# uricchio/2DSFS-scan

Measured on AMD Instinct MI355X. Metric: genomic windows/s (T2D+T1D+Fst) at 20 kb, n1=n2=50; HBM GB/s fraction, higher is better.
Workload: dtype f64

## Files before the change

### 2dsfs-scan_amd/csrc/sfs2d.hip

```cpp
#include <hip/hip_runtime.h>
#include <hip/hip_ext.h>

#include <algorithm>
#include <cmath>
#include <cstdint>
#include <cstdio>
#include <cstdlib>
#include <cstring>
#include <string>
#include <mutex>
#include <vector>

#include "sfs2d.h"
#include "sfs2d_kernels.hpp"

using namespace sfs2dk;

namespace {

struct PwTree {
  std::vector<int2> leaves;
  std::vector<int4> nodes;
  int nlevels = 0;
};
// ... 45 lines not shown

#define CTX_STREAM(c) ((c)->stream)

struct sfs2d_ctx {
  int device = 0;
  int ncu = 256;
  hipStream_t own = nullptr;
  hipStream_t stream = nullptr;
  double* d_lnx = nullptr;
  double* d_df = nullptr;
  hipEvent_t stagger = nullptr;
  std::string err;
  std::mutex err_mu;
};

struct sfs2d_data {
  sfs2d_ctx* ctx = nullptr;
  bool owned = false;
  uint32_t* counts = nullptr;
  uint32_t* pos = nullptr;
  uint16_t* ann = nullptr;
  long long* d_chrom_off = nullptr;
  int64_t n = 0;
  int32_t nchrom = 0;
  std::vector<int64_t> chrom_off;
  std::vector<uint32_t> last_pos;
  std::vector<uint32_t> host_pos;
  bool ann_owned = false;
  bool strict = true;
  uint32_t max_nc1 = 0xffffffffu, max_nc2 = 0xffffffffu;
  bool low_nc = true;
  unsigned long long* d_win_off = nullptr;
  uint32_t win_bp = 0, win_per_chrom = 0;
};

struct sfs2d_plan {
  sfs2d_ctx* ctx = nullptr;
  const sfs2d_data* data = nullptr;
  sfs2d_params prm{};
  KParams K{};
  int nbg = 0;
  bool do_bg = false, do_seg = false, lds_hist = true, bg_ready = false;
  bool seg_synth = false;
  bool seg_search = false;
  int64_t step = 0;
  bool fused = false;
  bool sliced = false;
  bool cnt = false;
  bool fst = false;
  double* d_fst = nullptr;
  double* d_fst_own = nullptr;
  unsigned long long* d_fsum = nullptr;
  int hr = 1;
  uint64_t runs = 0;
  int G = 64;
  bool gw = false;
  uint32_t* d_gscr = nullptr;
  int nscr = 0;
  bool p16 = true;
  size_t scan_lds = 0, bg_lds = 0, extra_lds = 0;
  int64_t nslots = 0, nrec = 0, extra_rec = -1;
  uint32_t last_chrom = 0;
  std::vector<Tile> tiles;
  std::vector<Chunk> chunks;
  std::vector<int4> slices;
  Tile* d_tiles = nullptr;
  Chunk* d_chunks = nullptr;
  uint2* d_slots = nullptr;
  uint32_t* d_repl = nullptr;
  uint32_t* d_bcount = nullptr;
  uint32_t* d_done = nullptr;
  uint32_t* d_ctr = nullptr;
  double* d_bgval = nullptr;
  PL* d_tab = nullptr;
  double* d_lp = nullptr;
  BgHead* d_head = nullptr;
  Bg1D* d_bg1d = nullptr;
// ... 217 lines not shown
template <bool B, bool S, bool L, bool N>
hipError_t launch_prep1(sfs2d_plan* pl) {
  const bool f = pl->K.ann_want >= 0 || pl->K.has_start || pl->K.has_end;
  return f ? launch_prep2<B, S, L, N, true>(pl) : launch_prep2<B, S, L, N, false>(pl);
}

hipError_t launch_prep_cnt(sfs2d_plan* pl) {
  const bool L = pl->lds_hist;
  const bool fs = pl->fst && !pl->fst_win && !pl->fst_scan;
  if (pl->do_bg && pl->do_seg)
    return L ? launch_prep1<true, true, true, false>(pl) : launch_prep1<true, true, false, false>(pl);
  if (pl->do_bg) return L ? launch_prep1<true, false, true, false>(pl) : launch_prep1<true, false, false, false>(pl);
  if (pl->do_seg) return launch_prep1<false, true, false, false>(pl);
  if (fs) return launch_prep1<false, false, false, false>(pl);
  return hipSuccess;
}

bool slots_only(const sfs2d_plan* pl) {
  return (pl->seg_synth || pl->seg_search) && pl->attached.empty() && !(pl->fst && !pl->fst_win && !pl->fst_scan);
}

hipError_t launch_slots_only(sfs2d_plan* pl) {
  const unsigned long long nw = (unsigned long long)pl->nslots;
  if (nw && pl->seg_synth)
    hipExtLaunchKernelGGL(k_slots_synth, dim3((unsigned)std::min<unsigned long long>(8192, (nw + 255) / 256)), dim3(256),
                          0, CTX_STREAM(pl->ctx), pl->kev[0], pl->kev[1], 0, pl->data->d_win_off, nw, pl->d_slots);
  else if (nw)
    hipExtLaunchKernelGGL(k_slots_search, dim3((unsigned)((nw + 255) / 256)), dim3(256), 0, CTX_STREAM(pl->ctx),
                          pl->kev[0], pl->kev[1], 0, pl->data->pos, pl->data->d_chrom_off, pl->d_slot_base,
                          pl->data->nchrom, (uint32_t)pl->prm.window, (uint32_t)nw, pl->d_slots);
  return hipGetLastError();
}

bool prep_runs(const sfs2d_plan* pl) {
  return !pl->tiles.empty() && (!pl->cnt || pl->do_bg || pl->do_seg || (pl->fst && !pl->fst_win && !pl->fst_scan));
}

hipError_t launch_slots_slide(sfs2d_plan* pl, bool ev) {
  const uint32_t ns = (uint32_t)pl->nslots;
  if (!ns) return hipSuccess;
  hipExtLaunchKernelGGL(k_slots_slide, dim3((ns + 255u) / 256u), dim3(256), 0, CTX_STREAM(pl->ctx), ev ? pl->kev[0] : nullptr,
                        ev ? pl->kev[1] : nullptr, 0, pl->data->pos, pl->data->d_chrom_off, pl->d_slot_base, pl->data->nchrom,
                        (uint32_t)pl->prm.window, (uint32_t)pl->step, ns, pl->d_slots);
  return hipGetLastError();
}

hipError_t launch_fst_win(sfs2d_plan* a) {
  const uint32_t ns = (uint32_t)a->nslots;
  if (!ns) return hipSuccess;
  const dim3 gf((unsigned)std::min<uint32_t>(2048u, (ns + 3u) / 4u));
  if (a->cnt)
    hipLaunchKernelGGL(k_fst_win<true>, gf, dim3(256), 0, CTX_STREAM(a->ctx), a->K, a->data->counts, scan_src(a), a->d_slots,
                       reinterpret_cast<const double2*>(a->ctx->d_df + 2 * LNT), a->d_fst, ns);
  else
    hipLaunchKernelGGL(k_fst_win<false>, gf, dim3(256), 0, CTX_STREAM(a->ctx), a->K, a->data->counts, scan_src(a), a->d_slots,
                       reinterpret_cast<const double2*>(a->ctx->d_df + 2 * LNT), a->d_fst, ns);
  return hipGetLastError();
}

hipError_t launch_prep(sfs2d_plan* pl, bool bins) {
  if (pl->tiles.empty()) return hipSuccess;
  const bool L = pl->lds_hist;
  if (!bins) return L ? launch_prep1<true, false, true, false>(pl) : launch_prep1<true, false, false, false>(pl);
  if (pl->cnt) return launch_prep_cnt(pl);
  if (pl->do_bg && pl->do_seg)
    return L ? launch_prep1<true, true, true, true>(pl) : launch_prep1<true, true, false, true>(pl);
// ... 307 lines not shown
  if (e != hipSuccess) {
    hipFree(d_woff);
    hipFree(d->counts); hipFree(d->pos); hipFree(d->ann); hipFree(d->d_chrom_off); delete d;
    return set_err(ctx, SFS2D_E_HIP, std::string("synthetic data: ") + hipGetErrorString(e));
  }
  d->d_win_off = d_woff;
  d->win_bp = sp->window_bp;
  d->win_per_chrom = sp->n_windows;
  d->last_pos.assign(sp->n_replicates, sp->n_windows * sp->window_bp);
  d->strict = true;
  d->max_nc1 = 2u * (uint32_t)sp->n1p;
  d->max_nc2 = 2u * (uint32_t)sp->n2p;
  *out = d;
  return 0;
}

int sfs2d_data_read(const sfs2d_data* d, uint32_t* counts, uint32_t* pos, int64_t n) {
  if (!d || n != d->n) return SFS2D_E_ARG;
  sfs2d_ctx* ctx = d->ctx;
  HIPCHK(ctx, hipSetDevice(ctx->device));
  HIPCHK(ctx, hipStreamSynchronize(CTX_STREAM(ctx)));
  if (counts && n) HIPCHK(ctx, hipMemcpy(counts, d->counts, sizeof(uint32_t) * (size_t)n, hipMemcpyDeviceToHost));
  if (pos && n) HIPCHK(ctx, hipMemcpy(pos, d->pos, sizeof(uint32_t) * (size_t)n, hipMemcpyDeviceToHost));
  return 0;
}

int sfs2d_data_free(sfs2d_data* d) {
  if (!d) return SFS2D_E_ARG;
  hipSetDevice(d->ctx->device);
  if (d->owned) { hipFree(d->counts); hipFree(d->pos); }
  if (d->owned || d->ann_owned) hipFree(d->ann);
  hipFree(d->d_chrom_off);
  hipFree(d->d_win_off);
  delete d;
  return 0;
}

static int make_kparams(sfs2d_ctx* ctx, const sfs2d_params* prm, int nchrom, KParams* K) {
  *K = KParams{};
  if (!prm) return set_err(ctx, SFS2D_E_ARG, "params is NULL");
  if (prm->n1p < 1 || prm->n2p < 1 || 2 * prm->n1p > 255 || 2 * prm->n2p > 255)
    return set_err(ctx, SFS2D_E_ARG, "pop sizes must satisfy 1 <= pop_size and 2*pop_size <= 255 (u8 counts)");
  if (prm->window_mode != SFS2D_WINDOW_BP && prm->window_mode != SFS2D_WINDOW_SNPS)
    return set_err(ctx, SFS2D_E_ARG, "bad window_mode");
  if (prm->window < 1 || prm->window > 0xffffffffll) return set_err(ctx, SFS2D_E_ARG, "window must be in [1, 2^32)");
  if (prm->bg_mode != SFS2D_BG_PER_CHROM && prm->bg_mode != SFS2D_BG_SUPPLIED) return set_err(ctx, SFS2D_E_ARG, "bad bg_mode");
  K->n1p = prm->n1p; K->n2p = prm->n2p; K->n1 = 2 * prm->n1p; K->n2 = 2 * prm->n2p;
  K->nb2 = (K->n1 + 1) * (K->n2 + 1);
  K->h1a = K->nb2; K->h1b = K->nb2 + K->n1 + 1; K->nh = (K->h1b + K->n2 + 1 + 3) & ~3;
  K->t1a = K->nb2; K->t1b = K->nb2 + K->n1p + 1; K->nt = K->t1b + K->n2p + 1;
  K->rtn = wl_rtn(K->n1p, K->n2p);
  K->fold = prm->fold ? 1 : 0;
  K->fold_thr = prm->fold ? K->n1p + K->n2p : 0x7fffffff;
  K->ann_want = prm->ann_want;
  K->has_start = prm->has_start ? 1 : 0; K->has_end = prm->has_end ? 1 : 0;
  K->start_pos = prm->start_pos; K->end_pos = prm->end_pos;
  K->ws = (unsigned)prm->window;
  div_magic(K->ws, &K->wmag, &K->wsh1, &K->wsh2);
  K->nchrom = nchrom;
  K->fst_e = 40;
  K->fst_scale = std::ldexp(1.0, K->fst_e);
  return 0;
}

static int plan_create(sfs2d_ctx* ctx, const sfs2d_data* data, const sfs2d_params* prm, int force_sliced, int64_t step,
                       sfs2d_plan** out);

// ... 193 lines not shown
        if (const char* ev = std::getenv("SFS2D_GW")) pl->gw = occ >= 1 && ev[0] == '1';
      }
      if (pl->gw) pl->scan_lds = gw_lds;
    }
  }
  if (pl->scan_lds > 160 * 1024) {
    delete pl;
    return set_err(ctx, SFS2D_E_ARG, "2D grid too large for LDS with 32-bit bins (windows of >= 65536 SNPs)");
  }
  const bool small = pl->do_bg && pl->G == WAVE;
  const double wpw = (double)pl->nslots / (2.0 * ctx->ncu * (SBLOCK / WAVE));
  pl->sliced = small && wpw < 4.0;
  if (const char* ev = std::getenv("SFS2D_FUSED")) pl->sliced = small && ev[0] == '0';
  if (force_sliced >= 0) pl->sliced = small && force_sliced == 1;
  pl->fused = small && !pl->sliced;
  pl->fst = (prm->flags & SFS2D_F_FST) != 0;
  pl->fst_scan = false;
  if (pl->fst && pl->cnt && pl->G == WAVE && !pl->gw) {
    const char* ev = std::getenv("SFS2D_FST_SCAN");
    pl->fst_scan = !(ev && ev[0] == '0');
    if (pl->fst_scan) {
      hipFuncAttributes fa{};
      const void* f = pl->p16 ? (const void*)k_scan_w<true, true, 2, true> : (const void*)k_scan_w<false, true, 2, true>;
      if (hipFuncGetAttributes(&fa, f) != hipSuccess || pl->scan_lds + fa.sharedSizeBytes > 160 * 1024) pl->fst_scan = false;
    }
  }
  pl->gate = pl->fst_scan && prm->fold && nc_ok;
  pl->lean = pl->gate && bp && K.n1p <= 31 && K.n2p <= 31;
  if (const char* ev = std::getenv("SFS2D_LEAN")) pl->lean = pl->lean && ev[0] != '0';
  const PwTree pw = pw_plan(K.nb2 - 3);
  pl->fst_mask = data->low_nc;
  pl->fst_win = pl->sliced && bp && pl->fst && !pl->fst_scan;
  if (slide) pl->fst_win = pl->fst && !pl->fst_scan;
  pl->nfst = pl->fst_win && !slide ? (int)std::min<int64_t>(1024, std::max<int64_t>(1, (pl->nslots + 7) / 8)) : 0;
  if (pl->scan_lds > 64 * 1024) {
    const int lds = (int)pl->scan_lds;
    const hipFuncAttribute A = hipFuncAttributeMaxDynamicSharedMemorySize;
    for (const void* f : {(const void*)k_scan_w<true, true, false, false>, (const void*)k_scan_w<false, true, false, false>,
                          (const void*)k_scan_w<true, false, false, false>, (const void*)k_scan_w<false, false, false, false>,
                          (const void*)k_scan_w<true, true, true, false>, (const void*)k_scan_w<false, true, true, false>,
                          (const void*)k_scan_w<true, false, true, false>, (const void*)k_scan_w<false, false, true, false>,
                          (const void*)k_scan_w<true, true, false, true>, (const void*)k_scan_w<false, true, false, true>,
                          (const void*)k_scan_w<true, false, false, true>, (const void*)k_scan_w<false, false, false, true>,
                          (const void*)k_scan_w<true, true, true, true>, (const void*)k_scan_w<false, true, true, true>,
                          (const void*)k_scan_w<true, false, true, true>, (const void*)k_scan_w<false, false, true, true>,
                          (const void*)k_scan_w<true, true, 2, true>, (const void*)k_scan_w<false, true, 2, true>,
                          (const void*)k_scan_w<true, false, 2, true>, (const void*)k_scan_w<false, false, 2, true>,
                          (const void*)k_scan_w<true, true, 3, true>, (const void*)k_scan_w<false, true, 3, true>,
                          (const void*)k_scan_w<true, false, 3, true>, (const void*)k_scan_w<false, false, 3, true>,
                          (const void*)k_scan_w<true, true, 2, true, true>, (const void*)k_scan_w<false, true, 2, true, true>,
                          (const void*)k_scan_w<true, false, 2, true, true>, (const void*)k_scan_w<false, false, 2, true, true>,
                          (const void*)k_scan_w<true, true, 3, true, true>, (const void*)k_scan_w<false, true, 3, true, true>,
                          (const void*)k_scan_w<true, false, 3, true, true>, (const void*)k_scan_w<false, false, 3, true, true>,
                          (const void*)k_scan_w<true, true, 2, true, true, true>, (const void*)k_scan_w<false, true, 2, true, true, true>,
                          (const void*)k_scan_w<true, false, 2, true, true, true>, (const void*)k_scan_w<false, false, 2, true, true, true>,
                          (const void*)k_scan_w<true, true, 3, true, true, true>, (const void*)k_scan_w<false, true, 3, true, true, true>,
                          (const void*)k_scan_w<true, false, 3, true, true, true>, (const void*)k_scan_w<false, false, 3, true, true, true>,
                          (const void*)k_scan_g<true, false, false>, (const void*)k_scan_g<false, false, false>,
                          (const void*)k_scan_g<true, true, false>, (const void*)k_scan_g<false, true, false>,
                          (const void*)k_scan_g<true, false, true>, (const void*)k_scan_g<false, false, true>,
                          (const void*)k_scan_g<true, true, true>, (const void*)k_scan_g<false, true, true>})
      hipFuncSetAttribute(f, A, lds);
  }
  if (pl->extra_lds > 64 * 1024) {
    for (const void* f : {(const void*)k_scan_extra<true, false>, (const void*)k_scan_extra<false, false>,
                          (const void*)k_scan_extra<true, true>, (const void*)k_scan_extra<false, true>})
// ... 157 lines not shown
    const int ke = jl == pl->nleaves ? K.nb2 : 1 + pw.leaves[jl].x;
    pl->slices.push_back(make_int4(kb, ke, j, jl));
  }
  if (pl->slices.empty()) pl->slices.push_back(make_int4(0, K.nb2, 0, 0));

  hipStream_t st = CTX_STREAM(ctx);
  rc = 0;
  rc = rc ? rc : dalloc(ctx, &pl->d_tiles, pl->tiles.size());
  rc = rc ? rc : dalloc(ctx, &pl->d_chunks, pl->chunks.size());
  rc = rc ? rc : dalloc(ctx, &pl->d_slots, (size_t)pl->nslots + 1);
  const size_t nrepl = pl->do_bg ? (size_t)(pl->fused ? 2 : 1) * REPL * nc * K.nh : 1;
  rc = rc ? rc : dalloc(ctx, &pl->d_repl, nrepl);
  rc = rc ? rc : dalloc(ctx, &pl->d_bcount, (size_t)2 * std::max(1, nc));
  rc = rc ? rc : dalloc(ctx, &pl->d_done, (size_t)pl->nbg);
  const size_t nctr = (size_t)2 * std::max(1, nc) * CTR_POOLS * CTR_STRIDE;
  rc = rc ? rc : dalloc(ctx, &pl->d_ctr, nctr);
  const size_t ngscr = pl->gw ? (size_t)pl->nscr * (K.nb2 + 1) : 0;
  if (pl->gw) rc = rc ? rc : dalloc(ctx, &pl->d_gscr, ngscr);
  rc = rc ? rc : dalloc(ctx, &pl->d_bgval, (size_t)pl->nbg * K.nt);
  rc = rc ? rc : dalloc(ctx, &pl->d_tab, (size_t)pl->nbg * K.nt);
  rc = rc ? rc : dalloc(ctx, &pl->d_lp, (size_t)pl->nbg * K.nt);
  rc = rc ? rc : dalloc(ctx, &pl->d_head, (size_t)pl->nbg);
  rc = rc ? rc : dalloc(ctx, &pl->d_bg1d, (size_t)pl->nbg);
  rc = rc ? rc : dalloc(ctx, &pl->d_leafsum, (size_t)pl->nbg * std::max(1, pl->nleaves));
  rc = rc ? rc : dalloc(ctx, &pl->d_leaves, pw.leaves.size());
  rc = rc ? rc : dalloc(ctx, &pl->d_nodes, pw.nodes.size());
  rc = rc ? rc : dalloc(ctx, &pl->d_slices, pl->slices.size());
  const size_t nbins = pl->cnt ? 4 : ((size_t)data->n + 3) / 4 * 4 + SCAN_PAD;
  rc = rc ? rc : dalloc(ctx, &pl->d_bins, nbins);
  rc = rc ? rc : dalloc(ctx, &pl->d_out, (size_t)pl->nrec);
  rc = rc ? rc : dalloc(ctx, &pl->d_err, 4);
  if (pl->fst) rc = rc ? rc : dalloc(ctx, &pl->d_fst, (size_t)pl->nslots + 1);
  pl->d_fst_own = pl->d_fst;
  if ((pl->seg_search || slide) && !rc) {
    std::vector<uint32_t> sb(pl->slot_base_h.begin(), pl->slot_base_h.end());
    rc = dalloc(ctx, &pl->d_slot_base, sb.size());
    if (!rc && hipMemcpy(pl->d_slot_base, sb.data(), sizeof(uint32_t) * sb.size(), hipMemcpyHostToDevice) != hipSuccess)
      rc = set_err(ctx, SFS2D_E_HIP, "slot bases upload");
  }
  if (pl->fst) rc = rc ? rc : dalloc(ctx, &pl->d_fsum, 2 * ((size_t)pl->nslots + 1));
  if (rc) { plan_free(pl); delete pl; return rc; }
  hipError_t e = hipSuccess;
#define PCPY(dst, v) if (e == hipSuccess && !(v).empty()) e = hipMemcpyAsync(dst, (v).data(), sizeof((v)[0]) * (v).size(), hipMemcpyHostToDevice, st)
  PCPY(pl->d_tiles, pl->tiles);
  PCPY(pl->d_chunks, pl->chunks);
  PCPY(pl->d_leaves, pw.leaves);
  PCPY(pl->d_nodes, pw.nodes);
  PCPY(pl->d_slices, pl->slices);
#undef PCPY
  if (e == hipSuccess) e = hipMemsetAsync(pl->d_slots, 0, sizeof(uint2) * ((size_t)pl->nslots + 1), st);
  if (e == hipSuccess && pl->do_bg) e = hipMemsetAsync(pl->d_repl, 0, sizeof(uint32_t) * nrepl, st);
  if (e == hipSuccess) e = hipMemsetAsync(pl->d_bcount, 0, sizeof(uint32_t) * 2 * std::max(1, nc), st);
  if (e == hipSuccess) e = hipMemsetAsync(pl->d_done, 0, sizeof(uint32_t) * pl->nbg, st);
  if (e == hipSuccess) e = hipMemsetAsync(pl->d_ctr, 0, sizeof(uint32_t) * nctr, st);
  if (e == hipSuccess && pl->gw) e = hipMemsetAsync(pl->d_gscr, 0, sizeof(uint32_t) * ngscr, st);
  if (e == hipSuccess) e = hipMemsetAsync(pl->d_err, 0, 4 * sizeof(uint32_t), st);
  if (e == hipSuccess) e = hipMemsetAsync(pl->d_bins, 0, sizeof(uint32_t) * nbins, st);
  if (e == hipSuccess && pl->fst) e = hipMemsetAsync(pl->d_fsum, 0, sizeof(unsigned long long) * 2 * ((size_t)pl->nslots + 1), st);
  if (e == hipSuccess) e = hipMemsetAsync(pl->d_out, 0, sizeof(sfs2d_window) * (size_t)pl->nrec, st);
  for (auto& ev : pl->ev) if (e == hipSuccess) e = hipEventCreate(&ev);
  if (e == hipSuccess) e = hipStreamSynchronize(st);
  if (e != hipSuccess) {
    plan_free(pl); delete pl;
    return set_err(ctx, SFS2D_E_HIP, std::string("plan setup: ") + hipGetErrorString(e));
  }
  pl->bg_ready = false;
  *out = pl;
// ... 20 lines not shown
  HIPCHK(ctx, hipStreamSynchronize(CTX_STREAM(ctx)));
  pl->bg_ready = true;
  return 0;
}

int sfs2d_plan_run_phase(sfs2d_plan* pl, int phase, sfs2d_window* out_dev) {
  if (!pl) return SFS2D_E_ARG;
  sfs2d_ctx* ctx = pl->ctx;
  if (pl->base) return set_err(ctx, SFS2D_E_ARG, "an attached plan runs with its base plan (sfs2d_plan_attach)");
  HIPCHK(ctx, hipSetDevice(ctx->device));
  hipEvent_t* te = nullptr;
  if (phase == 2) {
    te = pl->tpend;
    pl->tpend = nullptr;
  } else if (pl->timing && (pl->tseen++ % pl->tevery) == 0 && pl->tcount < pl->tmax) {
    te = &pl->tev[(size_t)pl->tcount * 6];
  }
  if (!pl->do_bg && !pl->bg_ready && phase != 1)
    return set_err(ctx, SFS2D_E_ARG, "supplied-background plan run before sfs2d_plan_set_background");
  for (int k = 0; k < 6; ++k) pl->kev[k] = (te && ((pl->tmask >> (k / 2)) & 1)) ? te[k] : nullptr;
  auto mark = [&](int k) -> int {
    if (te && ((pl->tmask >> (k / 2)) & 1)) {
      HIPCHK(ctx, hipEventRecord(te[k], CTX_STREAM(ctx)));
      HIPCHK(ctx, hipEventRecord(te[k + 1], CTX_STREAM(ctx)));
    }
    return 0;
  };
  int rc = 0;
  if (phase == 0 || phase == 1) {
    if (slots_only(pl)) {
      HIPCHK(ctx, launch_slots_only(pl));
      if (pl->nslots == 0 && (rc = mark(0))) return rc;
    } else {
      HIPCHK(ctx, launch_prep(pl, true));
      const bool slots = pl->step && pl->nslots;
      if (slots) HIPCHK(ctx, launch_slots_slide(pl, !prep_runs(pl)));
      if (!prep_runs(pl) && !slots && (rc = mark(0))) return rc;
    }
  }
  if (phase == 0 || phase == 2) {
    if (pl->do_bg && !pl->fused) HIPCHK(ctx, launch_bg_slices(pl));
    else if ((rc = mark(2))) return rc;
    if (pl->step && pl->fst_win) HIPCHK(ctx, launch_fst_win(pl));
    for (sfs2d_plan* a : pl->attached) HIPCHK(ctx, launch_attached(a));
    sfs2d_window* out = out_dev ? out_dev : pl->d_out;
    if (pl->chunks.empty() && (rc = mark(4))) return rc;
    HIPCHK(ctx, launch_scan_any(pl, out));
    pl->last_out = out;
    pl->runs++;
  }
  for (auto& e : pl->kev) e = nullptr;
  if (te && phase == 1) pl->tpend = te;
  else if (te) pl->tcount++;
  return 0;
}

int sfs2d_plan_grids(const sfs2d_plan* pl, int64_t* prep_threads, int64_t* scan_threads) {
  if (!pl) return SFS2D_E_ARG;
  if (prep_threads) *prep_threads = (int64_t)pl->tiles.size() * BLOCK1;
  if (scan_threads) *scan_threads = (int64_t)pl->chunks.size() * (pl->G == WAVE ? SBLOCK : pl->gw ? WAVE : BLOCK);
  return 0;
}

const char* sfs2d_plan_scan_kernel(const sfs2d_plan* pl) {
  if (!pl) return nullptr;
  if (pl->gw) return "k_scan_gw";
  return pl->G == WAVE ? "k_scan_w" : "k_scan_g";
}

int sfs2d_plan_scan_variant(const sfs2d_plan* pl, int* p16, int* fused, int* fst, int* cnt, int* gate, int* tri) {
  if (!pl) return SFS2D_E_ARG;
  if (!pl->variant_set) return set_err(pl->ctx, SFS2D_E_ARG, "sfs2d_plan_scan_variant: the plan has launched no scan kernel yet");
  int* const o[6] = {p16, fused, fst, cnt, gate, tri};
  for (int i = 0; i < 6; ++i)
    if (o[i]) *o[i] = pl->variant[i];
  return 0;
}

int sfs2d_plan_set_timing(sfs2d_plan* pl, int max_runs) { return sfs2d_plan_set_timing_sampled(pl, max_runs, 1); }

int sfs2d_plan_set_timing_sampled(sfs2d_plan* pl, int max_runs, int every) {
  return sfs2d_plan_set_timing_kernels(pl, max_runs, every, 7);
}

int sfs2d_plan_set_timing_kernels(sfs2d_plan* pl, int max_runs, int every, int kernel_mask) {
  if (!pl || max_runs < 0 || every < 1 || (kernel_mask & ~7) || !kernel_mask) return SFS2D_E_ARG;
  pl->tevery = every;
  pl->tmask = kernel_mask;
  pl->tseen = 0;
  sfs2d_ctx* ctx = pl->ctx;
  HIPCHK(ctx, hipStreamSynchronize(CTX_STREAM(ctx)));
  if ((size_t)max_runs * 6 > pl->tev.size()) {
    for (auto& e : pl->tev) if (e) hipEventDestroy(e);
    pl->tev.assign((size_t)max_runs * 6, nullptr);
    for (auto& e : pl->tev) HIPCHK(ctx, hipEventCreate(&e));
  }
  pl->tmax = max_runs;
  pl->tcount = 0;
  pl->tpend = nullptr;
  pl->timing = max_runs > 0;
// ... 429 lines not shown
  if (nrec == 0) return 0;
  int rc = null_tables(pl);
  if (rc) return rc;
  HIPCHK(ctx, hipMemcpyAsync(pl->d_ntask, pl->ntask_h.data(), sizeof(NullTask) * (size_t)ntasks, hipMemcpyHostToDevice, st));
  const uint2 key = make_uint2((uint32_t)np->seed, (uint32_t)(np->seed >> 32));
  const uint32_t blk = (uint32_t)block;
  if (maxm <= 65535u)
    return pl->cnt ? launch_null<true, true>(pl, np->replicates, nrec, key, blk, out)
                   : launch_null<true, false>(pl, np->replicates, nrec, key, blk, out);
  return pl->cnt ? launch_null<false, true>(pl, np->replicates, nrec, key, blk, out)
                 : launch_null<false, false>(pl, np->replicates, nrec, key, blk, out);
}

int sfs2d_plan_null_read(sfs2d_plan* pl, sfs2d_window* out_host, int64_t cap, int64_t* nrec_out) {
  if (!pl || !nrec_out) return SFS2D_E_ARG;
  sfs2d_ctx* ctx = pl->ctx;
  *nrec_out = pl->null_nrec;
  if (cap < pl->null_nrec) return set_err(ctx, SFS2D_E_CAP, "output capacity too small");
  if (pl->null_nrec && !out_host) return SFS2D_E_ARG;
  if (pl->null_nrec)
    HIPCHK(ctx, hipMemcpyAsync(out_host, pl->null_last, sizeof(sfs2d_window) * (size_t)pl->null_nrec, hipMemcpyDeviceToHost,
                               CTX_STREAM(ctx)));
  HIPCHK(ctx, hipStreamSynchronize(CTX_STREAM(ctx)));
  return 0;
}

int sfs2d_plan_time(sfs2d_plan* pl, int iters, double* ms_run, double* ms_k1, double* ms_k2, double* ms_k3) {
  if (!pl || iters < 1) return SFS2D_E_ARG;
  sfs2d_ctx* ctx = pl->ctx;
  hipStream_t st = CTX_STREAM(ctx);
  double t1 = 0, t2 = 0, t3 = 0, tall = 0;
  for (int it = 0; it < iters; ++it) {
    HIPCHK(ctx, hipEventRecord(pl->ev[0], st));
    HIPCHK(ctx, slots_only(pl) ? launch_slots_only(pl) : launch_prep(pl, true));
    if (pl->step) HIPCHK(ctx, launch_slots_slide(pl, false));
    HIPCHK(ctx, hipEventRecord(pl->ev[1], st));
    if (pl->do_bg && !pl->fused) HIPCHK(ctx, launch_bg_slices(pl));
    if (pl->step && pl->fst_win) HIPCHK(ctx, launch_fst_win(pl));
    for (sfs2d_plan* a : pl->attached) HIPCHK(ctx, launch_attached(a));
    HIPCHK(ctx, hipEventRecord(pl->ev[2], st));
    HIPCHK(ctx, launch_scan_any(pl, pl->d_out));
    pl->runs++;
    HIPCHK(ctx, hipEventRecord(pl->ev[3], st));
    HIPCHK(ctx, hipEventSynchronize(pl->ev[3]));
    float a = 0, b = 0, c = 0, d = 0;
    hipEventElapsedTime(&a, pl->ev[0], pl->ev[1]);
    hipEventElapsedTime(&b, pl->ev[1], pl->ev[2]);
    hipEventElapsedTime(&c, pl->ev[2], pl->ev[3]);
    hipEventElapsedTime(&d, pl->ev[0], pl->ev[3]);
    t1 += a; t2 += b; t3 += c; tall += d;
  }
  pl->last_out = pl->d_out;
  if (ms_run) *ms_run = tall / iters;
  if (ms_k1) *ms_k1 = t1 / iters;
  if (ms_k2) *ms_k2 = t2 / iters;
  if (ms_k3) *ms_k3 = t3 / iters;
  return 0;
}

int sfs2d_plan_destroy(sfs2d_plan* pl) {
  if (!pl) return SFS2D_E_ARG;
  hipSetDevice(pl->ctx->device);
  hipStreamSynchronize(CTX_STREAM(pl->ctx));
  for (sfs2d_plan* a : pl->attached) {
    a->base = pl;
    plan_free(a);
// ... 199 lines not shown
```

### 2dsfs-scan_amd/csrc/sfs2d_kernels.hpp

```cpp
#pragma once

#include <type_traits>
#include <hip/hip_runtime.h>

#include <cmath>
#include <cstdint>

#include "sfs2d.h"

namespace sfs2dk {

constexpr int WAVE = 64;
constexpr int BLOCK = 256;
constexpr int SBLOCK = 512;
constexpr int BLOCK1 = 512;
constexpr int FBLOCK = 1024;
constexpr int KBLOCK = 512;
constexpr int LNX_N = 1 << 20;
constexpr int LNT = 512;
constexpr int LNF = 256;
__host__ __device__ inline int wl_rtn(int n1p, int n2p) { return 2 * (n1p > n2p ? n1p : n2p) + 2; }
constexpr int RCPN = 512;
#ifndef SFS2D_ABL
#define SFS2D_ABL 0
// ... 2849 lines not shown
    else hi = mid;
  }
  const uint32_t j = s - slot_base[lo];
  const uint32_t cb = (uint32_t)chrom_off[lo], ce = (uint32_t)chrom_off[lo + 1];
  const uint32_t b = j ? lower_bound_pos(pos, cb, ce, (unsigned long long)j * ws + 1ull) : cb;
  const uint32_t e = lower_bound_pos(pos, b, ce, (unsigned long long)(j + 1) * ws + 1ull);
  slots[s] = b < e ? make_uint2(b + 1u, e) : make_uint2(0u, 0u);
}

__global__ __launch_bounds__(256) void k_slots_search(const uint32_t* __restrict__ pos,
                                                      const long long* __restrict__ chrom_off,
                                                      const uint32_t* __restrict__ slot_base, int nchrom, uint32_t ws,
                                                      uint32_t nslots, uint2* __restrict__ slots) {
  const uint32_t s = blockIdx.x * 256u + threadIdx.x;
  const uint32_t sc = min(s, nslots - 1u);
  int lo = 0, hi = nchrom;
  while (hi - lo > 1) {
    const int mid = (lo + hi) >> 1;
    if (slot_base[mid] <= sc) lo = mid;
    else hi = mid;
  }
  const uint32_t j = sc - slot_base[lo], ns = slot_base[lo + 1] - slot_base[lo];
  const uint32_t cb = (uint32_t)chrom_off[lo], ce = (uint32_t)chrom_off[lo + 1];
  auto lb = [&](uint32_t a, unsigned long long v) -> uint32_t { return lower_bound_pos(pos, a, ce, v); };
  const uint32_t b = j ? lb(cb, (unsigned long long)j * ws + 1ull) : cb;
  uint32_t e = __shfl_down(b, 1, WAVE);
  const bool lastw = j + 1u == ns;
  if (lastw) e = ce;
  else if ((threadIdx.x & (WAVE - 1)) == WAVE - 1 || s + 1u >= nslots)
    e = lb(b, (unsigned long long)(j + 1u) * ws + 1ull);
  if (s < nslots) slots[s] = b < e ? make_uint2(b + 1u, e) : make_uint2(0u, 0u);
}

__global__ __launch_bounds__(256) void k_slots_slide(const uint32_t* __restrict__ pos, const long long* __restrict__ chrom_off,
                                                     const uint32_t* __restrict__ slot_base, int nchrom, uint32_t ws,
                                                     uint32_t step, uint32_t nslots, uint2* __restrict__ slots) {
  const uint32_t s = blockIdx.x * 256u + threadIdx.x;
  if (s >= nslots) return;
  int lo = 0, hi = nchrom;
  while (hi - lo > 1) {
    const int mid = (lo + hi) >> 1;
    if (slot_base[mid] <= s) lo = mid;
    else hi = mid;
  }
  const uint32_t j = s - slot_base[lo];
  const uint32_t cb = (uint32_t)chrom_off[lo], ce = (uint32_t)chrom_off[lo + 1];
  const unsigned long long p0 = (unsigned long long)j * step;
  const uint32_t b = j ? lower_bound_pos(pos, cb, ce, p0 + 1ull) : cb;
  const uint32_t e = lower_bound_pos(pos, b, ce, p0 + (unsigned long long)ws + 1ull);
  slots[s] = b < e ? make_uint2(b + 1u, e) : make_uint2(0u, 0u);
}

__global__ __launch_bounds__(256) void k_fst_agg(const unsigned long long* __restrict__ bsum,
                                                 const uint32_t* __restrict__ bslot_base,
                                                 const uint32_t* __restrict__ slot_base, int nchrom, uint32_t m,
                                                 uint32_t nslots, int shift, unsigned long long* __restrict__ fsum) {
  const uint32_t s = blockIdx.x * 256u + threadIdx.x;
  if (s >= nslots) return;
  int lo = 0, hi = nchrom;
  while (hi - lo > 1) {
    const int mid = (lo + hi) >> 1;
    if (slot_base[mid] <= s) lo = mid;
    else hi = mid;
  }
  const uint32_t j = s - slot_base[lo];
  const uint32_t b0 = bslot_base[lo] + j * m, b1 = min(b0 + m, bslot_base[lo + 1]);
// ... 88 lines not shown
```

### 2dsfs-scan_amd/sfs2d/_lib.py

```python
from __future__ import annotations

import ctypes as C
import os

import numpy as np

HERE = os.path.dirname(os.path.abspath(__file__))
LIB_PATH = os.environ.get("SFS2D_LIB", os.path.join(HERE, "..", "csrc", "libsfs2d.so"))

OK = 0
E_ARG, E_HIP, E_NOMEM, E_KEY, E_GRID, E_CAP = -1, -2, -3, -4, -5, -6
WINDOW_BP, WINDOW_SNPS = 0, 1
BG_PER_CHROM, BG_SUPPLIED = 0, 1
F_PREV_EXTRA = 1
F_FST = 2
W_EMPTY = 0x80000000
W_BG2_ZERO, W_BG1A_ZERO, W_BG1B_ZERO = 0x1, 0x2, 0x4
W_EXTRA = 0x40000000


def bg_row_words(n1p: int, n2p: int) -> int:
    return (2 * n1p + 1) * (2 * n2p + 1) + 2 * n1p + 2 * n2p + 3

EXPORTS = [
    "sfs2d_abi_version", "sfs2d_ctx_create", "sfs2d_ctx_destroy", "sfs2d_last_error", "sfs2d_ctx_set_stream",
    "sfs2d_data_upload", "sfs2d_data_wrap_device", "sfs2d_data_free", "sfs2d_bg_hist", "sfs2d_plan_create",
    "sfs2d_plan_num_records", "sfs2d_plan_set_background", "sfs2d_plan_run", "sfs2d_plan_run_many", "sfs2d_plan_set_timing_sampled",
    "sfs2d_plan_set_timing_kernels",
    "sfs2d_plan_fst_read", "sfs2d_plan_fst_buffer", "sfs2d_plan_read",
    "sfs2d_plan_bg_buffer", "sfs2d_plan_bg_words", "sfs2d_plan_bg_exchange", "sfs2d_plan_run_phase", "sfs2d_plan_check", "sfs2d_plan_time",
    "sfs2d_plan_destroy", "sfs2d_scan", "sfs2d_plan_set_timing", "sfs2d_plan_timing_read",
    "sfs2d_plan_stats", "sfs2d_plan_grids", "sfs2d_plan_scan_kernel", "sfs2d_plan_attach", "sfs2d_data_synth_sims",
    "sfs2d_data_read", "sfs2d_plan_run_streams", "sfs2d_ctx_use_own_stream", "sfs2d_bg_hist_dev", "sfs2d_plan_bg_rows_dev", "sfs2d_plan_bg_rows_set_dev",
    "sfs2d_ctx_get_stream", "sfs2d_plan_set_fst_out", "sfs2d_graph_create", "sfs2d_graph_launch", "sfs2d_graph_destroy",
    "sfs2d_plan_create_sliding", "sfs2d_plan_attach_sliding", "sfs2d_plan_null_run", "sfs2d_plan_null_read",
    "sfs2d_plan_null_run_blocks",
    "sfs2d_plan_scan_variant",
]
ABI_VERSION = 2


class Sfs2dError(RuntimeError):
    def __init__(self, code, msg):
        super().__init__(f"sfs2d error {code}: {msg}")
        self.code = code


class SynthParams(C.Structure):
    _fields_ = [("seed", C.c_uint64), ("generation", C.c_uint32), ("n_replicates", C.c_uint32),
                ("n_windows", C.c_uint32), ("window_bp", C.c_uint32), ("n1p", C.c_int32), ("n2p", C.c_int32)]


class NullParams(C.Structure):
    _fields_ = [("seed", C.c_uint64), ("replicates", C.c_uint32)]


class Params(C.Structure):
    _fields_ = [
        ("n1p", C.c_int32), ("n2p", C.c_int32), ("fold", C.c_int32), ("window_mode", C.c_int32),
        ("window", C.c_int64), ("bg_mode", C.c_int32), ("ann_want", C.c_int32),
        ("has_start", C.c_int32), ("has_end", C.c_int32), ("start_pos", C.c_int64), ("end_pos", C.c_int64),
        ("flags", C.c_uint32), ("scan_wgs_per_cu", C.c_uint32),
    ]


WINDOW_DTYPE = np.dtype([
    ("chrom", "<u4"), ("wid", "<u4"), ("begin", "<u4"), ("end", "<u4"), ("snp_count", "<u4"),
    ("n2", "<u4"), ("n2_all", "<u4"), ("n1a", "<u4"), ("n1b", "<u4"), ("flags", "<u4"),
    ("t2d", "<f8"), ("t1d_p1", "<f8"), ("t1d_p2", "<f8"),
])
# ... 30 lines not shown
    L.sfs2d_data_free.argtypes = [vp]
    L.sfs2d_bg_hist.argtypes = [vp, vp, C.POINTER(Params), i32, vp, vp, vp]
    L.sfs2d_plan_create.argtypes = [vp, vp, C.POINTER(Params), C.POINTER(vp)]
    L.sfs2d_plan_num_records.argtypes = [vp]
    L.sfs2d_plan_num_records.restype = i64
    L.sfs2d_plan_set_background.argtypes = [vp, vp, vp, vp]
    L.sfs2d_plan_run.argtypes = [vp, vp]
    L.sfs2d_plan_run_many.argtypes = [vp, C.c_int, vp]
    L.sfs2d_plan_run_streams.argtypes = [vp, vp, vp, C.c_int, C.c_int]
    L.sfs2d_graph_create.argtypes = [vp, vp, vp, C.c_int, C.c_int, C.POINTER(vp)]
    L.sfs2d_graph_launch.argtypes = [vp, C.c_int]
    L.sfs2d_graph_destroy.argtypes = [vp]
    L.sfs2d_plan_set_timing_sampled.argtypes = [vp, C.c_int, C.c_int]
    L.sfs2d_plan_set_timing_kernels.argtypes = [vp, C.c_int, C.c_int, C.c_int]
    L.sfs2d_plan_fst_read.argtypes = [vp, vp, i64]
    L.sfs2d_plan_fst_buffer.argtypes = [vp, C.POINTER(vp), C.POINTER(i64)]
    L.sfs2d_plan_run_phase.argtypes = [vp, C.c_int, vp]
    L.sfs2d_plan_read.argtypes = [vp, vp, i64, C.POINTER(i64)]
    L.sfs2d_plan_bg_buffer.argtypes = [vp, C.POINTER(vp), C.POINTER(i64)]
    L.sfs2d_plan_bg_words.argtypes = [vp, C.POINTER(i64), C.POINTER(i64), C.POINTER(i64)]
    L.sfs2d_plan_bg_exchange.argtypes = [vp, vp, vp, C.c_int]
    L.sfs2d_bg_hist_dev.argtypes = [vp, vp, C.POINTER(Params), i32, vp]
    L.sfs2d_plan_bg_rows_dev.argtypes = [vp, vp, i64]
    L.sfs2d_plan_bg_rows_set_dev.argtypes = [vp, vp, i64]
    L.sfs2d_plan_check.argtypes = [vp]
    L.sfs2d_plan_time.argtypes = [vp, C.c_int] + [C.POINTER(C.c_double)] * 4
    L.sfs2d_plan_destroy.argtypes = [vp]
    L.sfs2d_plan_set_timing.argtypes = [vp, C.c_int]
    L.sfs2d_plan_stats.argtypes = [vp, C.POINTER(C.c_uint32)]
    L.sfs2d_plan_grids.argtypes = [vp, C.POINTER(i64), C.POINTER(i64)]
    L.sfs2d_plan_scan_kernel.argtypes = [vp]
    L.sfs2d_plan_scan_kernel.restype = C.c_char_p
    L.sfs2d_plan_scan_variant.argtypes = [vp] + [C.POINTER(C.c_int)] * 6
    L.sfs2d_plan_attach.argtypes = [vp, C.POINTER(Params), C.POINTER(vp)]
    L.sfs2d_plan_create_sliding.argtypes = [vp, vp, C.POINTER(Params), i64, C.POINTER(vp)]
    L.sfs2d_plan_attach_sliding.argtypes = [vp, C.POINTER(Params), i64, C.POINTER(vp)]
    L.sfs2d_plan_null_run.argtypes = [vp, C.POINTER(NullParams), vp, i64, vp]
    L.sfs2d_plan_null_run_blocks.argtypes = [vp, C.POINTER(NullParams), i64, vp, i64, vp]
    L.sfs2d_plan_null_read.argtypes = [vp, vp, i64, C.POINTER(i64)]
    L.sfs2d_data_synth_sims.argtypes = [vp, C.POINTER(SynthParams), vp, vp, i32, vp, i32, C.POINTER(vp)]
    L.sfs2d_data_read.argtypes = [vp, vp, vp, i64]
    L.sfs2d_ctx_use_own_stream.argtypes = [vp]
    L.sfs2d_ctx_get_stream.argtypes = [vp, C.POINTER(vp)]
    L.sfs2d_plan_set_fst_out.argtypes = [vp, vp]
    L.sfs2d_plan_timing_read.argtypes = [vp, C.POINTER(C.c_int)] + [C.POINTER(C.c_double)] * 3
    L.sfs2d_scan.argtypes = [vp, vp, C.POINTER(Params), vp, vp, vp, vp, i64, C.POINTER(i64)]
    _lib = L
    return L


def ptr(a: np.ndarray):
    return a.ctypes.data_as(C.c_void_p) if a is not None else None
```

### 2dsfs-scan_amd/sfs2d/engine.py

```python
from __future__ import annotations

import ctypes as C
from dataclasses import dataclass
from typing import Optional

import numpy as np

from . import _lib as L
from .pack import PackedSNPs


@dataclass
class ScanConfig:
    n1p: int
    n2p: int
    fold: bool = True
    window_mode: int = L.WINDOW_BP
    window: int = 20000
    bg_mode: int = L.BG_PER_CHROM
    ann_want: int = -1
    start_position: Optional[int] = None
    end_position: Optional[int] = None
    prev_extra: bool = False
    fst: bool = False
# ... 252 lines not shown
    def _null_read_call(self) -> np.ndarray:
        n = C.c_int64()
        out = np.zeros(self._null_call_n, dtype=L.WINDOW_DTYPE)
        self.eng.check(self.eng.lib.sfs2d_plan_null_read(self.h, L.ptr(out) if len(out) else None, len(out), C.byref(n)))
        return out

    def null_read(self) -> np.ndarray:
        if getattr(self, "_null_dev", False):
            raise ValueError("the last null_run wrote to the caller's device buffer")
        parts = getattr(self, "_null_parts", None)
        if parts is None:
            raise ValueError("null_read before null_run")
        return np.concatenate(parts) if parts else self._null_read_call()

    def bg_buffer(self):
        p = C.c_void_p()
        nb = C.c_int64()
        self.eng.check(self.eng.lib.sfs2d_plan_bg_buffer(self.h, C.byref(p), C.byref(nb)))
        return p.value, nb.value

    def time(self, iters: int = 10):
        v = [C.c_double() for _ in range(4)]
        self.eng.check(self.eng.lib.sfs2d_plan_time(self.h, iters, *[C.byref(x) for x in v]))
        return tuple(x.value for x in v)

    def grids(self):
        a, b = C.c_int64(), C.c_int64()
        self.eng.check(self.eng.lib.sfs2d_plan_grids(self.h, C.byref(a), C.byref(b)))
        return a.value, b.value

    def scan_kernel(self) -> str:
        return self.eng.lib.sfs2d_plan_scan_kernel(self.h).decode()

    def scan_variant(self) -> dict:
        v = [C.c_int() for _ in range(6)]
        self.eng.check(self.eng.lib.sfs2d_plan_scan_variant(self.h, *[C.byref(x) for x in v]))
        return dict(zip(("p16", "fused", "fst", "cnt", "gate", "tri"), (x.value for x in v)))

    def stats(self) -> int:
        v = C.c_uint32()
        self.eng.check(self.eng.lib.sfs2d_plan_stats(self.h, C.byref(v)))
        return int(v.value)

    def set_timing(self, max_runs: int, every: int = 1, kernels: int = 7):
        self.eng.check(self.eng.lib.sfs2d_plan_set_timing_kernels(self.h, int(max_runs), int(every), int(kernels)))

    def timing_read(self):
        n = C.c_int()
        v = [C.c_double() for _ in range(3)]
        self.eng.check(self.eng.lib.sfs2d_plan_timing_read(self.h, C.byref(n), *[C.byref(x) for x in v]))
        return n.value, tuple(x.value for x in v)

    def close(self):
        if self.h:
            for a in self.attached:
                a.h = C.c_void_p()
            self.attached = []
            if self.base is not None and self in self.base.attached:
                self.base.attached.remove(self)
            self.eng.lib.sfs2d_plan_destroy(self.h)
            self.h = C.c_void_p()

    def __del__(self):
        try:
            self.close()
        except Exception:
# ... 76 lines not shown
```

### include/sfs2d.h

```cpp
#ifndef SFS2D_H
#define SFS2D_H

#include <stdint.h>

#ifdef __cplusplus
extern "C" {
#endif

#define SFS2D_ABI_VERSION 2

#define SFS2D_OK 0
#define SFS2D_E_ARG (-1)
#define SFS2D_E_HIP (-2)
#define SFS2D_E_NOMEM (-3)
#define SFS2D_E_KEY (-4)
#define SFS2D_E_GRID (-5)
#define SFS2D_E_CAP (-6)

#define SFS2D_WINDOW_BP 0
#define SFS2D_WINDOW_SNPS 1

#define SFS2D_BG_PER_CHROM 0
#define SFS2D_BG_SUPPLIED 1

// ... 72 lines not shown
int sfs2d_plan_create(sfs2d_ctx* ctx, const sfs2d_data* data, const sfs2d_params* params, sfs2d_plan** out);
int64_t sfs2d_plan_num_records(const sfs2d_plan* plan);
int sfs2d_plan_set_background(sfs2d_plan* plan, const double* bg2d, const double* bg1a, const double* bg1b);
int sfs2d_plan_run(sfs2d_plan* plan, sfs2d_window* out_dev);
int sfs2d_plan_run_many(sfs2d_plan* plan, int nruns, sfs2d_window* out_dev);
int sfs2d_plan_run_streams(sfs2d_plan* const* plans, void* const* streams, sfs2d_window* const* outs, int nplans,
                           int nruns);
int sfs2d_graph_create(sfs2d_plan* const* plans, void* const* streams, sfs2d_window* const* outs, int nplans,
                       int nruns, sfs2d_graph** out);
int sfs2d_graph_launch(sfs2d_graph* graph, int nlaunch);
int sfs2d_graph_destroy(sfs2d_graph* graph);
int sfs2d_plan_read(sfs2d_plan* plan, sfs2d_window* out_host, int64_t cap, int64_t* nrec_out);
int sfs2d_plan_bg_buffer(sfs2d_plan* plan, void** dev_ptr, int64_t* nbytes);
int sfs2d_plan_bg_words(const sfs2d_plan* plan, int64_t* replicas, int64_t* nchrom, int64_t* bins);
int sfs2d_plan_bg_exchange(sfs2d_plan* plan, uint32_t* host_repl, uint32_t* host_sums, int to_device);
int sfs2d_plan_bg_rows_dev(sfs2d_plan* plan, int64_t* d_rows, int64_t row_stride);
int sfs2d_plan_bg_rows_set_dev(sfs2d_plan* plan, const int64_t* d_rows, int64_t row_stride);
int sfs2d_plan_fst_read(sfs2d_plan* plan, double* out_host, int64_t cap);
int sfs2d_plan_fst_buffer(sfs2d_plan* plan, void** dev_ptr, int64_t* nslots);
int sfs2d_plan_set_fst_out(sfs2d_plan* plan, double* d_fst);
int sfs2d_plan_run_phase(sfs2d_plan* plan, int phase, sfs2d_window* out_dev);
int sfs2d_plan_attach(sfs2d_plan* base, const sfs2d_params* params, sfs2d_plan** out);
int sfs2d_plan_create_sliding(sfs2d_ctx* ctx, const sfs2d_data* data, const sfs2d_params* params, int64_t step,
                              sfs2d_plan** out);
int sfs2d_plan_attach_sliding(sfs2d_plan* base, const sfs2d_params* params, int64_t step, sfs2d_plan** out);
typedef struct { uint64_t seed; uint32_t replicates; } sfs2d_null_params;
int sfs2d_plan_null_run(sfs2d_plan* plan, const sfs2d_null_params* np, const int64_t* tasks, int64_t ntasks,
                        sfs2d_window* out_dev);
int sfs2d_plan_null_run_blocks(sfs2d_plan* plan, const sfs2d_null_params* np, int64_t block, const int64_t* tasks,
                               int64_t ntasks, sfs2d_window* out_dev);
int sfs2d_plan_null_read(sfs2d_plan* plan, sfs2d_window* out_host, int64_t cap, int64_t* nrec_out);
int sfs2d_plan_grids(const sfs2d_plan* plan, int64_t* prep_threads, int64_t* scan_threads);
const char* sfs2d_plan_scan_kernel(const sfs2d_plan* plan);
int sfs2d_plan_scan_variant(const sfs2d_plan* plan, int* p16, int* fused, int* fst, int* cnt, int* gate, int* tri);
int sfs2d_plan_stats(sfs2d_plan* plan, uint32_t* exact_windows);
int sfs2d_plan_check(sfs2d_plan* plan);
int sfs2d_plan_set_timing(sfs2d_plan* plan, int max_runs);
int sfs2d_plan_set_timing_sampled(sfs2d_plan* plan, int max_samples, int every);
int sfs2d_plan_set_timing_kernels(sfs2d_plan* plan, int max_samples, int every, int kernel_mask);
int sfs2d_plan_timing_read(sfs2d_plan* plan, int* nruns, double* ms_k1, double* ms_k2, double* ms_k3);
int sfs2d_plan_time(sfs2d_plan* plan, int iters, double* ms_per_run, double* ms_k1, double* ms_k2, double* ms_k3);
int sfs2d_plan_destroy(sfs2d_plan* plan);

int sfs2d_scan(sfs2d_ctx* ctx, const sfs2d_data* data, const sfs2d_params* params, const double* bg2d,
               const double* bg1a, const double* bg1b, sfs2d_window* out_host, int64_t cap, int64_t* nrec_out);

#ifdef __cplusplus
}
#endif
#endif
```

Before: 927.2 million.

## Build cached position index to compute window slot bounds without prep segmentation

Adds a per-dataset coarse position index, built once on the device and cached with a mutex, that maps bucketed bp positions to SNP offsets. A new slot kernel uses it to find window boundaries with short bounded searches, sharing each boundary between neighbouring lanes through a wave shuffle. When the plan uses bp windows with counts and background, this path replaces the segmentation work in prep (do_seg is cleared). The cost is extra device memory, a one-time index build with a host sync, and an added small kernel launch on each run.

```diff
diff --git a/2dsfs-scan_amd/csrc/sfs2d.hip b/2dsfs-scan_amd/csrc/sfs2d.hip
--- a/2dsfs-scan_amd/csrc/sfs2d.hip
+++ b/2dsfs-scan_amd/csrc/sfs2d.hip
@@ -101,6 +101,10 @@
   bool low_nc = true;
   unsigned long long* d_win_off = nullptr;
   uint32_t win_bp = 0, win_per_chrom = 0;
+  mutable std::mutex pidx_mu;
+  mutable uint32_t* d_pidx = nullptr;
+  mutable uint32_t* d_pidx_base = nullptr;
+  mutable uint32_t* d_pidx_sh = nullptr;
 };
 
 struct sfs2d_plan {
@@ -112,6 +116,7 @@
   bool do_bg = false, do_seg = false, lds_hist = true, bg_ready = false;
   bool seg_synth = false;
   bool seg_search = false;
+  bool seg_index = false;
   int64_t step = 0;
   bool fused = false;
   bool sliced = false;
@@ -395,6 +400,17 @@
   return hipGetLastError();
 }
 
+hipError_t launch_slots_index(sfs2d_plan* pl) {
+  const uint32_t ns = (uint32_t)pl->nslots;
+  if (!ns) return hipSuccess;
+  const sfs2d_data* d = pl->data;
+  hipExtLaunchKernelGGL(k_slots_index, dim3((ns + 255u) / 256u), dim3(256), 0, CTX_STREAM(pl->ctx), pl->kev[0], nullptr, 0,
+                        d->pos, d->d_chrom_off, pl->d_slot_base, d->d_pidx, d->d_pidx_base, d->d_pidx_sh, d->nchrom,
+                        (uint32_t)pl->prm.window, ns, pl->d_slots);
+  pl->kev[0] = nullptr;
+  return hipGetLastError();
+}
+
 bool prep_runs(const sfs2d_plan* pl) {
   return !pl->tiles.empty() && (!pl->cnt || pl->do_bg || pl->do_seg || (pl->fst && !pl->fst_win && !pl->fst_scan));
 }
@@ -768,7 +784,50 @@
   if (d->owned || d->ann_owned) hipFree(d->ann);
   hipFree(d->d_chrom_off);
   hipFree(d->d_win_off);
+  hipFree(d->d_pidx); hipFree(d->d_pidx_base); hipFree(d->d_pidx_sh);
   delete d;
+  return 0;
+}
+
+static int data_pos_index(sfs2d_ctx* ctx, const sfs2d_data* d) {
+  std::lock_guard<std::mutex> g(d->pidx_mu);
+  if (d->d_pidx) return 0;
+  const int nc = d->nchrom;
+  std::vector<uint32_t> base(nc + 1, 0), sh(std::max(1, nc), 0);
+  unsigned long long nent = 0;
+  for (int c = 0; c < nc; ++c) {
+    const int64_t len = d->chrom_off[c + 1] - d->chrom_off[c];
+    if (len > 0) {
+      const unsigned long long want = (unsigned long long)std::max<int64_t>(1, len / 16);
+      uint32_t s = 0;
+      while (((unsigned long long)d->last_pos[c] >> s) + 1ull > want) ++s;
+      sh[c] = s;
+      nent += ((unsigned long long)d->last_pos[c] >> s) + 2ull;
+    }
+    base[c + 1] = (uint32_t)nent;
+  }
+  if (nent > 0xffffffffull) return set_err(ctx, SFS2D_E_ARG, "position index too large");
+  uint32_t *idx = nullptr, *db = nullptr, *ds = nullptr;
+  int rc = dalloc(ctx, &idx, (size_t)nent);
+  rc = rc ? rc : dalloc(ctx, &db, base.size());
+  rc = rc ? rc : dalloc(ctx, &ds, sh.size());
+  hipError_t e = hipSuccess;
+  if (!rc) {
+    hipStream_t st = CTX_STREAM(ctx);
+    e = hipMemcpyAsync(db, base.data(), sizeof(uint32_t) * base.size(), hipMemcpyHostToDevice, st);
+    if (e == hipSuccess) e = hipMemcpyAsync(ds, sh.data(), sizeof(uint32_t) * sh.size(), hipMemcpyHostToDevice, st);
+    if (e == hipSuccess && nent) {
+      hipLaunchKernelGGL(k_pos_index, dim3((unsigned)((nent + 255) / 256)), dim3(256), 0, st, d->pos, d->d_chrom_off, db, ds,
+                         nc, (uint32_t)nent, idx);
+      e = hipGetLastError();
+    }
+    if (e == hipSuccess) e = hipStreamSynchronize(st);
+  }
+  if (rc || e != hipSuccess) {
+    hipFree(idx); hipFree(db); hipFree(ds);
+    return rc ? rc : set_err(ctx, SFS2D_E_HIP, std::string("position index: ") + hipGetErrorString(e));
+  }
+  d->d_pidx = idx; d->d_pidx_base = db; d->d_pidx_sh = ds;
   return 0;
 }
 
@@ -1028,6 +1087,12 @@
   pl->fst_mask = data->low_nc;
   pl->fst_win = pl->sliced && bp && pl->fst && !pl->fst_scan;
   if (slide) pl->fst_win = pl->fst && !pl->fst_scan;
+  pl->seg_index = bp && !slide && pl->cnt && pl->do_bg && !seg_prep && force_sliced < 0 && data->owned &&
+                  !(pl->fst && !pl->fst_win && !pl->fst_scan);
+  if (pl->seg_index) {
+    if ((rc = data_pos_index(ctx, data))) { delete pl; return rc; }
+    pl->do_seg = false;
+  }
   pl->nfst = pl->fst_win && !slide ? (int)std::min<int64_t>(1024, std::max<int64_t>(1, (pl->nslots + 7) / 8)) : 0;
   if (pl->scan_lds > 64 * 1024) {
     const int lds = (int)pl->scan_lds;
@@ -1251,7 +1316,7 @@
   rc = rc ? rc : dalloc(ctx, &pl->d_err, 4);
   if (pl->fst) rc = rc ? rc : dalloc(ctx, &pl->d_fst, (size_t)pl->nslots + 1);
   pl->d_fst_own = pl->d_fst;
-  if ((pl->seg_search || slide) && !rc) {
+  if ((pl->seg_search || pl->seg_index || slide) && !rc) {
     std::vector<uint32_t> sb(pl->slot_base_h.begin(), pl->slot_base_h.end());
     rc = dalloc(ctx, &pl->d_slot_base, sb.size());
     if (!rc && hipMemcpy(pl->d_slot_base, sb.data(), sizeof(uint32_t) * sb.size(), hipMemcpyHostToDevice) != hipSuccess)
@@ -1338,6 +1403,7 @@
       HIPCHK(ctx, launch_slots_only(pl));
       if (pl->nslots == 0 && (rc = mark(0))) return rc;
     } else {
+      if (pl->seg_index) HIPCHK(ctx, launch_slots_index(pl));
       HIPCHK(ctx, launch_prep(pl, true));
       const bool slots = pl->step && pl->nslots;
       if (slots) HIPCHK(ctx, launch_slots_slide(pl, !prep_runs(pl)));
@@ -1372,6 +1438,15 @@
   if (!pl) return nullptr;
   if (pl->gw) return "k_scan_gw";
   return pl->G == WAVE ? "k_scan_w" : "k_scan_g";
+}
+
+const char* sfs2d_plan_seg_kind(const sfs2d_plan* pl) {
+  if (!pl) return nullptr;
+  if (pl->base) return pl->step ? "slide" : pl->prm.window_mode == SFS2D_WINDOW_BP ? "bp" : "none";
+  if (pl->step) return "slide";
+  if (pl->seg_index) return "index";
+  if (slots_only(pl)) return pl->seg_synth ? "synth" : "search";
+  return pl->do_seg ? "prep" : "none";
 }
 
 int sfs2d_plan_scan_variant(const sfs2d_plan* pl, int* p16, int* fused, int* fst, int* cnt, int* gate, int* tri) {
@@ -1867,6 +1942,7 @@
   double t1 = 0, t2 = 0, t3 = 0, tall = 0;
   for (int it = 0; it < iters; ++it) {
     HIPCHK(ctx, hipEventRecord(pl->ev[0], st));
+    if (pl->seg_index) HIPCHK(ctx, launch_slots_index(pl));
     HIPCHK(ctx, slots_only(pl) ? launch_slots_only(pl) : launch_prep(pl, true));
     if (pl->step) HIPCHK(ctx, launch_slots_slide(pl, false));
     HIPCHK(ctx, hipEventRecord(pl->ev[1], st));
diff --git a/2dsfs-scan_amd/csrc/sfs2d_kernels.hpp b/2dsfs-scan_amd/csrc/sfs2d_kernels.hpp
--- a/2dsfs-scan_amd/csrc/sfs2d_kernels.hpp
+++ b/2dsfs-scan_amd/csrc/sfs2d_kernels.hpp
@@ -2905,6 +2905,56 @@
   if (s < nslots) slots[s] = b < e ? make_uint2(b + 1u, e) : make_uint2(0u, 0u);
 }
 
+__global__ __launch_bounds__(256) void k_pos_index(const uint32_t* __restrict__ pos, const long long* __restrict__ chrom_off,
+                                                   const uint32_t* __restrict__ ibase, const uint32_t* __restrict__ sh,
+                                                   int nchrom, uint32_t nent, uint32_t* __restrict__ idx) {
+  const uint32_t e = blockIdx.x * 256u + threadIdx.x;
+  if (e >= nent) return;
+  int lo = 0, hi = nchrom;
+  while (hi - lo > 1) {
+    const int mid = (lo + hi) >> 1;
+    if (ibase[mid] <= e) lo = mid;
+    else hi = mid;
+  }
+  const uint32_t k = e - ibase[lo], cells = ibase[lo + 1] - ibase[lo] - 1u;
+  const uint32_t cb = (uint32_t)chrom_off[lo], ce = (uint32_t)chrom_off[lo + 1];
+  idx[e] = k == 0u ? cb : k >= cells ? ce : lower_bound_pos(pos, cb, ce, ((unsigned long long)k << sh[lo]) + 1ull);
+}
+
+__device__ __forceinline__ void slots_index(uint32_t s, const uint32_t* __restrict__ pos,
+                                            const long long* __restrict__ chrom_off, const uint32_t* __restrict__ slot_base,
+                                            const uint32_t* __restrict__ idx, const uint32_t* __restrict__ ibase,
+                                            const uint32_t* __restrict__ sh, int nchrom, uint32_t ws, uint32_t nslots,
+                                            uint2* __restrict__ slots) {
+  const uint32_t sc = min(s, nslots - 1u);
+  int lo = 0, hi = nchrom;
+  while (hi - lo > 1) {
+    const int mid = (lo + hi) >> 1;
+    if (slot_base[mid] <= sc) lo = mid;
+    else hi = mid;
+  }
+  const uint32_t j = sc - slot_base[lo], ns = slot_base[lo + 1] - slot_base[lo];
+  const uint32_t cb = (uint32_t)chrom_off[lo], ce = (uint32_t)chrom_off[lo + 1];
+  const uint32_t ib = ibase[lo], cells = ibase[lo + 1] - ib - 1u, shc = sh[lo];
+  auto bound = [&](uint32_t jj) -> uint32_t {
+    const unsigned long long p = (unsigned long long)jj * ws, k = p >> shc;
+    if (k >= (unsigned long long)cells) return ce;
+    return lower_bound_pos(pos, idx[ib + (uint32_t)k], idx[ib + (uint32_t)k + 1u], p + 1ull);
+  };
+  const uint32_t b = j ? bound(j) : cb;
+  uint32_t e = __shfl_down(b, 1, WAVE);
+  if (j + 1u == ns) e = ce;
+  else if ((threadIdx.x & (WAVE - 1)) == WAVE - 1 || s + 1u >= nslots) e = bound(j + 1u);
+  if (s < nslots) slots[s] = b < e ? make_uint2(b + 1u, e) : make_uint2(0u, 0u);
+}
+
+__global__ __launch_bounds__(256) void k_slots_index(const uint32_t* __restrict__ pos, const long long* __restrict__ chrom_off,
+                                                     const uint32_t* __restrict__ slot_base, const uint32_t* __restrict__ idx,
+                                                     const uint32_t* __restrict__ ibase, const uint32_t* __restrict__ sh,
+                                                     int nchrom, uint32_t ws, uint32_t nslots, uint2* __restrict__ slots) {
+  slots_index(blockIdx.x * 256u + threadIdx.x, pos, chrom_off, slot_base, idx, ibase, sh, nchrom, ws, nslots, slots);
+}
+
 __global__ __launch_bounds__(256) void k_slots_slide(const uint32_t* __restrict__ pos, const long long* __restrict__ chrom_off,
                                                      const uint32_t* __restrict__ slot_base, int nchrom, uint32_t ws,
                                                      uint32_t step, uint32_t nslots, uint2* __restrict__ slots) {
diff --git a/2dsfs-scan_amd/sfs2d/_lib.py b/2dsfs-scan_amd/sfs2d/_lib.py
--- a/2dsfs-scan_amd/sfs2d/_lib.py
+++ b/2dsfs-scan_amd/sfs2d/_lib.py
@@ -35,7 +35,7 @@
     "sfs2d_ctx_get_stream", "sfs2d_plan_set_fst_out", "sfs2d_graph_create", "sfs2d_graph_launch", "sfs2d_graph_destroy",
     "sfs2d_plan_create_sliding", "sfs2d_plan_attach_sliding", "sfs2d_plan_null_run", "sfs2d_plan_null_read",
     "sfs2d_plan_null_run_blocks",
-    "sfs2d_plan_scan_variant",
+    "sfs2d_plan_scan_variant", "sfs2d_plan_seg_kind",
 ]
 ABI_VERSION = 2
 
@@ -132,6 +132,8 @@
     L.sfs2d_plan_scan_kernel.argtypes = [vp]
     L.sfs2d_plan_scan_kernel.restype = C.c_char_p
     L.sfs2d_plan_scan_variant.argtypes = [vp] + [C.POINTER(C.c_int)] * 6
+    L.sfs2d_plan_seg_kind.argtypes = [vp]
+    L.sfs2d_plan_seg_kind.restype = C.c_char_p
     L.sfs2d_plan_attach.argtypes = [vp, C.POINTER(Params), C.POINTER(vp)]
     L.sfs2d_plan_create_sliding.argtypes = [vp, vp, C.POINTER(Params), i64, C.POINTER(vp)]
     L.sfs2d_plan_attach_sliding.argtypes = [vp, C.POINTER(Params), i64, C.POINTER(vp)]
diff --git a/2dsfs-scan_amd/sfs2d/engine.py b/2dsfs-scan_amd/sfs2d/engine.py
--- a/2dsfs-scan_amd/sfs2d/engine.py
+++ b/2dsfs-scan_amd/sfs2d/engine.py
@@ -308,6 +308,9 @@
     def scan_kernel(self) -> str:
         return self.eng.lib.sfs2d_plan_scan_kernel(self.h).decode()
 
+    def seg_kind(self) -> str:
+        return self.eng.lib.sfs2d_plan_seg_kind(self.h).decode()
+
     def scan_variant(self) -> dict:
         v = [C.c_int() for _ in range(6)]
         self.eng.check(self.eng.lib.sfs2d_plan_scan_variant(self.h, *[C.byref(x) for x in v]))
diff --git a/include/sfs2d.h b/include/sfs2d.h
--- a/include/sfs2d.h
+++ b/include/sfs2d.h
@@ -128,6 +128,7 @@
 int sfs2d_plan_null_read(sfs2d_plan* plan, sfs2d_window* out_host, int64_t cap, int64_t* nrec_out);
 int sfs2d_plan_grids(const sfs2d_plan* plan, int64_t* prep_threads, int64_t* scan_threads);
 const char* sfs2d_plan_scan_kernel(const sfs2d_plan* plan);
+const char* sfs2d_plan_seg_kind(const sfs2d_plan* plan);
 int sfs2d_plan_scan_variant(const sfs2d_plan* plan, int* p16, int* fused, int* fst, int* cnt, int* gate, int* tri);
 int sfs2d_plan_stats(sfs2d_plan* plan, uint32_t* exact_windows);
 int sfs2d_plan_check(sfs2d_plan* plan);
```

After: 983.3 million, median of 6. 6.1% higher.
